# Jhuighuy/StormRuler

Measured on AMD Instinct MI355X. Metric: CG iterations/sec, 256^3 Poisson per GPU (+ SpMV achieved HBM GB/s in `roofline`), higher is better.
Workload: dtype f64

## Files before the change

### stormruler_amd/csrc/common.hpp

```cpp
#pragma once

#include <hip/hip_runtime.h>

#include <cstdint>
#include <cstdio>
#include <string>
#include <unordered_map>
#include <vector>

#include "../../include/storm_hip.h"

namespace storm {

void set_error(const char *fmt, ...) __attribute__((format(printf, 1, 2)));

#define STORM_FAIL(code, ...)        \
  do {                               \
    ::storm::set_error(__VA_ARGS__); \
    return (code);                   \
  } while (0)

#define STORM_REQUIRE(cond, ...) \
  do {                           \
    if (!(cond)) STORM_FAIL(STORM_HIP_E_INVALID, __VA_ARGS__); \
// ... 138 lines not shown
  int64_t opt_profile_spmv = 0;
  std::vector<storm::LazyStmt> lazy_q;
  std::unordered_map<const void *, int> occupancy;
  int64_t opt_test_disable = 0;
  int64_t opt_lazy = 0;
  int callback_depth = 0;
  int64_t n_lazy_fused_dots = 0, n_lazy_fused_pairs = 0, n_lazy_apply_dots = 0, n_lazy_cg_steps = 0;
  storm_hip_vec *lazy_spare = nullptr;
  int64_t opt_profile_comm = 0;
  int64_t opt_blas1_nt = 1;
  static constexpr int64_t opt_blas1_nt_rows = (int64_t)6 << 20;
  static constexpr int64_t opt_graph = 0;
  static constexpr int64_t opt_coop_mgs_min_rows = 0;
  int64_t opt_coop_mgs = 1;
  int64_t opt_latency_publish = 1;
  int64_t opt_coop_plain = 1;
  int64_t opt_coop_force_fail = 0;
  int coop_ran = 0;
  int coop_disabled = 0;
  int coop_fallback = 0;
  int64_t coop_skip = 0, coop_backoff = 0;
  int64_t opt_latency_path = 1;
  int64_t opt_resident_path = 1;
  static constexpr int64_t opt_resident_min_rows = 0;
  int64_t opt_resident_max_rows = (int64_t)1 << 22;
  int64_t opt_resident_planes = 0;
  static constexpr int64_t opt_resident_max_planes = 12;
  char *d_res_exch = nullptr;
  int64_t res_exch_rows = 0;
  int64_t opt_resident_profile = 0;
  long long *d_res_prof = nullptr;
  int res_prof_blocks = 0;
  char *d_res_slots = nullptr;
  int opt_lin_fuse = 1;
  int64_t opt_ticket_verify_inject = 0;
  int64_t opt_ticket_verify = 0;
  int opt_ticket_reduce = 1;
  int opt_fused_reduce = 1;
  int opt_latency_cache = 1;
  int64_t opt_latency_rows = 1 << 19;
  int64_t opt_rccl_fused = 1;
  int64_t opt_rccl_ticket = 1;
  int64_t opt_comm_wait_seconds = 120;
  int64_t opt_rccl_flag_wait = 1;
  int64_t opt_rccl_early_halo = 1;
  static constexpr int64_t opt_ipc_bicg_ticket = 1;
  static constexpr int64_t opt_ipc_fused = 1;
  static constexpr int64_t opt_ipc_streams = 2;
  int64_t opt_generic_solvers = 0;
  int64_t opt_cg_march_fill = 2048;
  int64_t opt_cg_march_alternate = 1;
  int64_t opt_cg_march = 8;
  int64_t opt_cg_residual_march = 1;
  int64_t opt_cg_fuse = 1;
  std::vector<std::pair<size_t, double *>> pool;
  struct VecArena {
    char *base = nullptr;
    size_t bytes = 0, pitch = 0;
    int slots = 0, used = 0;
  };
  std::vector<VecArena> arenas;
  int64_t opt_vec_arena = 1;
  static constexpr int64_t opt_vec_arena_contiguous = 1;
  static constexpr int64_t opt_cg_roles = 8;
  static constexpr int64_t opt_vec_arena_slots = 8;
  static constexpr int64_t opt_vec_arena_max_bytes = (int64_t)64 << 30;
  static constexpr int64_t opt_vec_arena_skew_kib = 0;
  size_t pool_bytes = 0;
  int64_t opt_pool_bytes = (int64_t)16 << 30;
  std::vector<hipEvent_t> prof_events;
  size_t prof_used = 0;
  const int *api_done = nullptr;
  int64_t n_resident_solves = 0, n_latency_solves = 0, n_throughput_solves = 0, n_engine_solves = 0, n_cg_fused_steps = 0;
  int64_t n_cg_residual_marches = 0;
  int64_t n_mgs_chain_steps = 0, n_mgs_quad_steps = 0;
  storm::Comm *comm = nullptr;
  int n_ranks = 1, rank = 0;
};

struct storm_hip_vec {
  storm_hip_ctx *ctx = nullptr;
  int64_t n_owned = 0, n_halo = 0;
  double *d = nullptr;
  double *base = nullptr;
  size_t bytes = 0;
  bool exposed = false;
};
constexpr int kVecGuard = 32;

namespace storm {

struct HaloPlan {
  int n_nbrs = 0;
  std::vector<int> nbr_rank;
  std::vector<int64_t> send_ptr, recv_ptr;
  int *d_send_idx = nullptr;
  double *d_sendbuf = nullptr;
  int64_t n_send = 0;
};

}

struct storm_hip_op {
  storm_hip_ctx *ctx = nullptr;
  int64_t n_rows = 0, n_halo = 0;
  int64_t n_slices = 0, n_interior_slices = 0;
  int64_t nnz = 0, ell_slots = 0, max_row_len = 0;
  int64_t *d_slice_off = nullptr;
  char *d_pack = nullptr;
  double *d_dict = nullptr;
  int dict_size = 0;
  int *d_offs = nullptr;
  int offs_size = 0;
  int xcd_group_sell = 0;
  int pair = 0;
  uint8_t *d_rec_idx = nullptr;
  uint64_t *d_rec_words = nullptr;
  int rec_words = 0;
  char *d_bnd_pack = nullptr;
  int bnd_width = 0;
  int canon_k = 0, canon_m1 = -1;
  int canon_off[7] = {0, 0, 0, 0, 0, 0, 0};
  int64_t pack_bytes = 0;
  int64_t spw = 1;
  int64_t tail_rows = 0, tail_nnz = 0;
  int *d_tail_row = nullptr;
  int64_t *d_tail_ptr = nullptr;
// ... 147 lines not shown
```

### stormruler_amd/csrc/context.hip

```cpp
#include <cstdarg>
#include <cstring>
#include <random>

#include <algorithm>
#include "common.hpp"

#include <cstddef>

namespace storm {

static thread_local char g_error[1024] = "";

void set_error(const char *fmt, ...) {
  va_list ap;
  va_start(ap, fmt);
  vsnprintf(g_error, sizeof g_error, fmt, ap);
  va_end(ap);
}

}

using namespace storm;

static void pool_release(storm_hip_ctx *c);
// ... 138 lines not shown
  else if (!strcmp(key, "coop_mgs_lds")) c->opt_coop_mgs_lds = value;
  else if (!strcmp(key, "coop_mgs_quad")) c->opt_coop_mgs_quad = value;
  else if (!strcmp(key, "cg_march_fill")) c->opt_cg_march_fill = value;
  else if (!strcmp(key, "resident_early")) c->opt_resident_early = value;
  else if (!strcmp(key, "mgs_steps")) c->opt_mgs_steps = value;
  else if (!strcmp(key, "vec_arena")) c->opt_vec_arena = value;
  else if (!strcmp(key, "spmv_mixed")) c->opt_spmv_mixed = value;
  else if (!strcmp(key, "spmv_canon_tile")) c->opt_spmv_canon_tile = value;
  else if (!strcmp(key, "spmv_canon_tile_min_rows")) c->opt_spmv_canon_tile_min_rows = value;
  else if (!strcmp(key, "fused_reduce")) c->opt_fused_reduce = (int)value;
  else if (!strcmp(key, "ticket_reduce")) c->opt_ticket_reduce = (int)value;
  else if (!strcmp(key, "ticket_verify")) c->opt_ticket_verify = value;
  else if (!strcmp(key, "ticket_verify_inject")) c->opt_ticket_verify_inject = value;
  else if (!strcmp(key, "lin_fuse")) c->opt_lin_fuse = (int)value;
  else if (!strcmp(key, "latency_rows")) c->opt_latency_rows = value;
  else if (!strcmp(key, "latency_cache")) c->opt_latency_cache = (int)value;
  else if (!strcmp(key, "nontemporal")) c->opt_nt = value;
  else if (!strcmp(key, "spmv_dict")) c->opt_spmv_dict = value;
  else if (!strcmp(key, "pool_bytes")) {
    c->opt_pool_bytes = value;
    if ((int64_t)c->pool_bytes > value || (value == 0 && !c->pool.empty())) {
      (void)hipStreamSynchronize(c->stream);
      pool_release(c);
    }
  }
  else if (!strcmp(key, "spmv_spw")) c->opt_spmv_spw = value;
  else if (!strcmp(key, "spmv_xcd_remap")) {
    STORM_REQUIRE(value >= 0 && value <= 4096, "ctx_set_option: spmv_xcd_remap %lld (0 .. 4096)", (long long)value);
    c->opt_spmv_xcd_remap = c->opt_spmv_xcd_remap_sell = value;
  }
  else if (!strcmp(key, "test_disable")) {
    c->opt_test_disable = value;
    c->opt_coop_mgs_apply = !(value & 1), c->opt_coop_mgs_prefetch = c->opt_coop_mgs_lds_prefetch = !(value & 2);
    c->opt_resident_apply_cache = !(value & 4), c->opt_resident_halo_interleave = !(value & 8);
    c->opt_latency_publish = !(value & 16), c->opt_coop_plain = !(value & 32), c->opt_cg_march_alternate = !(value & 64);
    c->opt_coop_mgs_xcd_runs = !(value & 128), c->opt_coop_mgs_alternate = !(value & 256);
    c->opt_coop_mgs_rotate_early = !(value & 512);
  }
  else if (!strcmp(key, "lazy_statements")) {
    if (value == 0) {
      STORM_TRY(lazy_sync(c));
      if (c->lazy_spare) (void)storm_hip_vec_destroy(c->lazy_spare), c->lazy_spare = nullptr;
    }
    c->opt_lazy = value;
  }
  else if (!strcmp(key, "profile_spmv")) c->opt_profile_spmv = value;
  else if (!strcmp(key, "profile_comm")) {
    c->opt_profile_comm = value;
    if (value != 0) STORM_TRY(comm_profile_reset(c));
  }
  else if (!strcmp(key, "cg_fuse")) c->opt_cg_fuse = value;
  else if (!strcmp(key, "cg_march")) c->opt_cg_march = value;
  else if (!strcmp(key, "cg_residual_march")) c->opt_cg_residual_march = value;
  else if (!strcmp(key, "spmv_record_index")) c->opt_spmv_record_index = value;
  else if (!strcmp(key, "blas1_nt")) c->opt_blas1_nt = value;
  else STORM_FAIL(STORM_HIP_E_INVALID, "ctx_set_option: unknown key '%s'", key);
  return STORM_HIP_OK;
}

int storm_hip_ctx_get_counter(storm_hip_ctx *c, const char *key, int64_t *value) {
  STORM_REQUIRE(c && key && value, "ctx_get_counter: null argument");
  if (!strcmp(key, "resident_solves")) *value = c->n_resident_solves;
  else if (!strcmp(key, "latency_solves")) *value = c->n_latency_solves;
  else if (!strcmp(key, "throughput_solves")) *value = c->n_throughput_solves;
  else if (!strcmp(key, "engine_solves")) *value = c->n_engine_solves;
  else if (!strcmp(key, "cg_fused_steps")) *value = c->n_cg_fused_steps;
  else if (!strcmp(key, "cg_residual_marches")) *value = c->n_cg_residual_marches;
  else if (!strcmp(key, "mgs_chain_steps")) *value = c->n_mgs_chain_steps;
  else if (!strcmp(key, "mgs_quad_steps")) *value = c->n_mgs_quad_steps;
  else if (!strcmp(key, "lazy_fused_dots")) *value = c->n_lazy_fused_dots;
  else if (!strcmp(key, "lazy_fused_pairs")) *value = c->n_lazy_fused_pairs;
  else if (!strcmp(key, "lazy_apply_dots")) *value = c->n_lazy_apply_dots;
  else if (!strcmp(key, "lazy_cg_steps")) *value = c->n_lazy_cg_steps;
  else if (!strcmp(key, "lazy_waiting")) *value = (int64_t)c->lazy_q.size();
  else if (!strncmp(key, "ipc_", 4)) {
    static const char *names[6] = {"ipc_allreduce_wait_ticks", "ipc_allreduces", "ipc_ack_wait_ticks", "ipc_ack_waits",
                                   "ipc_halo_slow_poll_ticks", "ipc_halo_slow_polls"};
    int k = -1;
    for (int i = 0; i < 6; ++i)
      if (!strcmp(key, names[i])) k = i;
    STORM_REQUIRE(k >= 0, "ctx_get_counter: unknown key '%s'", key);
    const long long v = comm_ipc_stat(c, k);
    STORM_REQUIRE(v >= 0, "ctx_get_counter: '%s' needs the peer-window transport", key);
    *value = v;
  }
  else if (!strncmp(key, "rccl_prof_", 10)) {
    static const char *names[8] = {"rccl_prof_exchanges", "rccl_prof_event_to_comm_ticks", "rccl_prof_pack_ticks",
                                   "rccl_prof_sendrecv_ticks", "rccl_prof_unhidden_wait_ticks", "rccl_prof_resume_ticks",
                                   "rccl_prof_allreduces", "rccl_prof_allreduce_ticks"};
    int k = -1;
    for (int i = 0; i < 8; ++i)
      if (!strcmp(key, names[i])) k = i;
    STORM_REQUIRE(k >= 0, "ctx_get_counter: unknown key '%s'", key);
    const long long v = comm_profile_read(c, k);
    STORM_REQUIRE(v >= 0, "ctx_get_counter: '%s' needs the RCCL transport with option profile_comm = 1", key);
    *value = v;
  }
  else if (!strncmp(key, "resident_phase_max_", 19) || !strncmp(key, "resident_phase_mean_", 20)) {
    const bool mx = key[15] == 'm' && key[16] == 'a';
    const int k = atoi(key + (mx ? 19 : 20));
    STORM_REQUIRE(c->d_res_prof != nullptr && c->res_prof_blocks > 0 && k >= 0 && k < 8, "ctx_get_counter: no resident profile (option resident_profile)");
    std::vector<long long> h((size_t)c->res_prof_blocks * 8);
    HIP_TRY(hipStreamSynchronize(c->stream));
    HIP_TRY(hipMemcpy(h.data(), c->d_res_prof, sizeof(long long) * h.size(), hipMemcpyDeviceToHost));
    long long m = 0, sum = 0;
    for (int b = 0; b < c->res_prof_blocks; ++b) m = std::max(m, h[(size_t)b * 8 + k]), sum += h[(size_t)b * 8 + k];
    *value = mx ? m : sum / c->res_prof_blocks;
  } else if (!strncmp(key, "resident_phase_block_", 21)) {
    int b = 0, k = 0;
    STORM_REQUIRE(sscanf(key + 21, "%d_%d", &b, &k) == 2 && c->d_res_prof != nullptr && b >= 0 && b < c->res_prof_blocks && k >= 0 && k < 8,
                  "ctx_get_counter: no such block / phase");
    long long v = 0;
    HIP_TRY(hipStreamSynchronize(c->stream));
    HIP_TRY(hipMemcpy(&v, c->d_res_prof + (size_t)b * 8 + k, sizeof v, hipMemcpyDeviceToHost));
    *value = v;
  }
  else STORM_FAIL(STORM_HIP_E_INVALID, "ctx_get_counter: unknown key '%s'", key);
  return STORM_HIP_OK;
}

// ... 395 lines not shown
```

### stormruler_amd/csrc/solver_device.hpp

```cpp
#pragma once

#include "common.hpp"
#include "ipc_device.hpp"
#include "wave_device.hpp"

namespace storm {

__device__ __forceinline__ double safe_divide(double x, double y) { return (y == 0.0) ? 0.0 : (x / y); }

__device__ inline void advance(SolverState *st, double abs_err) {
  st->absolute_error = abs_err;
  st->relative_error = abs_err / st->initial_error;
  bool conv = false;
  conv |= (st->abs_tol > 0.0) && (st->absolute_error < st->abs_tol);
  conv |= (st->rel_tol > 0.0) && (st->relative_error < st->rel_tol);
  st->iteration += 1;
  if (st->history) st->history[st->iteration] = abs_err;
  if (conv) st->converged = 1;
  if (conv || st->iteration >= st->num_iterations) st->done = 1;
  if (st->done_ring)
    __hip_atomic_store(st->done_ring + (st->iteration - 1) % kStateRing,
                       ring_word(st->ring_gen, (unsigned long long)st->iteration, st->done != 0), __ATOMIC_RELAXED,
                       __HIP_MEMORY_SCOPE_SYSTEM);
}

__device__ inline void begin(SolverState *st, double initial_error) {
  st->initial_error = initial_error;
  st->absolute_error = initial_error;
  st->relative_error = 0.0;
  st->iteration = 0;
  st->converged = 0;
  st->done = 0;
  if (st->history) st->history[0] = initial_error;
  if (st->abs_tol > 0.0 && initial_error < st->abs_tol) st->converged = 1, st->done = 1;
  if (st->num_iterations <= 0) st->done = 1;
  if (st->done && st->done_ring)
    for (int i = 0; i < kStateRing; ++i)
      __hip_atomic_store(st->done_ring + i, ring_word(st->ring_gen, kRingIterMask, true), __ATOMIC_RELAXED, __HIP_MEMORY_SCOPE_SYSTEM);
}

struct GmresDev {
  double *H, *beta, *cs, *sn;
  int m;
};
__device__ inline void gmres_givens_update(SolverState *st, GmresDev g, int k, double hn) {
  const int m = g.m;
#define H_(i, j) g.H[(i) * m + (j)]
  H_(k + 1, k) = hn;
  for (int i = 0; i < k; ++i) {
    const double chi = g.cs[i] * H_(i, k) + g.sn[i] * H_(i + 1, k);
    H_(i + 1, k) = -g.sn[i] * H_(i, k) + g.cs[i] * H_(i + 1, k);
    H_(i, k) = chi;
  }
  const double a = H_(k, k), b = H_(k + 1, k);
  const double rr = hypot(a, b);
  double cs, sn;
  if (rr > 0.0) cs = a / rr, sn = b / rr;
  else cs = 1.0, sn = 0.0;
  g.cs[k] = cs, g.sn[k] = sn;
  H_(k, k) = cs * H_(k, k) + sn * H_(k + 1, k);
  H_(k + 1, k) = 0.0;
  g.beta[k + 1] = -sn * g.beta[k];
  g.beta[k] *= cs;
  advance(st, fabs(g.beta[k + 1]));
#undef H_
}

__device__ __forceinline__ double block_sum256(double v, double *lds4) {
  v = wave_sum_down(v);
  const int lane = threadIdx.x & (kWave - 1), wave = threadIdx.x >> 6;
  __syncthreads();
  if (lane == 0) lds4[wave] = v;
  __syncthreads();
  return (lds4[0] + lds4[1]) + (lds4[2] + lds4[3]);
}

__device__ __forceinline__ double block_fold(const double *__restrict__ p, int i0, int i1, double *lds4) {
  double v = 0.0;
#pragma unroll 8
  for (int i = i0 + threadIdx.x; i < i1; i += kBlock) v += p[i];
  return block_sum256(v, lds4);
}
__device__ __forceinline__ double block_fold(const double *__restrict__ p, int n, double *lds4) {
  return block_fold(p, 0, n, lds4);
}

template <int K>
struct OutPtrs {
  double *p[K];
};

template <class Epi, int K>
__global__ __launch_bounds__(kBlock) void reduce_finish_kernel(const double *__restrict__ partials, int nblocks, int k,
                                                               OutPtrs<K> out, const int *done, IpcDev w, int use_ipc, Epi epi) {
  if (done && *done) return;
  __shared__ double lds4[4];
  __shared__ double vals[K];
  for (int j = 0; j < k; ++j) {
    const double sum = block_fold(partials + (int64_t)j * nblocks, nblocks, lds4);
    if (threadIdx.x == 0) vals[j] = sum;
  }
  if (use_ipc) ipc_allreduce_block(w, vals, k);
  else __syncthreads();
  if ((int)threadIdx.x < k) *out.p[threadIdx.x] = vals[threadIdx.x];
  __syncthreads();
  if (threadIdx.x == 0) epi();
}

template <class Epi, int K, class Tail>
int k_reduce_finish(storm_hip_ctx *c, const double *partials, int nblocks, int k, const OutPtrs<K> &out, const int *done,
                    const Epi &epi, const OutPtrs<K> &local, Tail rccl_tail) {
  STORM_TRY(k_reduce_stage1(c, &partials, &nblocks, k, done));
  IpcDev w{};
  const bool one = c->comm == nullptr || comm_ipc_next(c, &w);
  hipLaunchKernelGGL((reduce_finish_kernel<Epi, K>), dim3(1), dim3(kBlock), 0, c->stream, partials, nblocks, k, one ? out : local,
                     done, w, (int)(c->comm != nullptr && one), one ? epi : Epi{});
  HIP_TRY(hipGetLastError());
  return one ? STORM_HIP_OK : rccl_tail();
}

}
```

### stormruler_amd/csrc/solvers.hip

```cpp
#include <algorithm>
#include <cmath>
#include <cstddef>
#include <cstring>

#include "common.hpp"
#include "blas1_device.hpp"
#include "wave_device.hpp"
#include "solver_device.hpp"
#include "ticket_device.hpp"
#include "ipc_device.hpp"
#include "spmv_device.hpp"

namespace storm {

enum Slot {
  S_GAMMA = 0, S_PZ, S_GAMMA_NEW, S_BETA, S_ALPHA,
  S_RHO, S_RTV, S_TR, S_TT, S_OMEGA, S_RR, S_RHO_NEW,
  S_TMP, S_HN,
  S_SCRATCH = 32,
  S_ALPHA_SEEN = 48,
};

enum StepKind {
  STEP_NONE = 0,
// ... 265 lines not shown
      el[u] = 0.0;
      if (lane == 0) el[u] = one_at(row - 1);
      if (lane == kWave - 1) el[u] = one_at(row + 2);
    }
#pragma unroll
    for (int u = 0; u < kUnroll; ++u) {
      const int64_t i = base + u * kBlock;
      double2v xg[6];
      xg[0] = nb[u][0], xg[1] = nb[u][1], xg[4] = nb[u][2], xg[5] = nb[u][3];
      const double left = dpp_shift<0x138>(c[u].y);
      const double right = dpp_shift<0x130>(c[u].x);
      xg[2].x = lane == 0 ? el[u] : left;
      xg[2].y = c[u].x;
      xg[3].x = c[u].y;
      xg[3].y = lane == kWave - 1 ? el[u] : right;
      const double2v vz = lattice_pair_apply(dict_sh, rec_word<IDX>(w[u], words_sh), xg, c[u], op_alpha, op_beta);
      if (i < n2) {
        vr[u] -= alpha * vz;
        r2[i] = vr[u];
        acc += vr[u].x * vr[u].x;
        acc += vr[u].y * vr[u].y;
      }
    }
  }
  cg_r_finish(st, acc, bx, nullptr, tickets, IpcDev{}, 0, lds4);
}

static bool cg_r_recompute_applies(const storm_hip_op *op, bool tick) {
  storm_hip_ctx *c = op->ctx;
  MarchArgs M;
  int nb = 0;
  return c->opt_cg_residual_march != 0 && tick && c->comm == nullptr && c->opt_ticket_verify == 0 && op->n_rows % 2 == 0 &&
         spmv_can_march(op) && cg_march_geometry(op, &M, &nb);
}
static int cg_r_recompute_run(const storm_hip_op *op, int nbv, Scal alpha, Scal beta, const double *p, SolverState *st, double *r,
                              const double *pz_partials, int n_pz, int reverse) {
  storm_hip_ctx *c = op->ctx;
  CanonTileArgs T;
  int nbt = 0;
  STORM_REQUIRE(canon_tile_geometry(op, &T, &nbt), "cg: the residual recompute needs a lattice operator");
  const SellArgs A = lattice_args(op);
  const size_t lds = sizeof(uint64_t) * (size_t)A.rec_words_n;
  const TicketArgs tk{c->d_tickets, c->d_partials, c->d_ticket_sums};
  if (A.rec_idx != nullptr)
    hipLaunchKernelGGL(cg_r_recompute_kernel<true>, dim3(nbv), dim3(kBlock), lds, c->stream, op->n_rows, st, r, p, A, T, alpha,
                       beta, pz_partials, n_pz, reverse, tk);
  else
    hipLaunchKernelGGL(cg_r_recompute_kernel<false>, dim3(nbv), dim3(kBlock), lds, c->stream, op->n_rows, st, r, p, A, T, alpha,
                       beta, pz_partials, n_pz, reverse, tk);
  HIP_TRY(hipGetLastError());
  return STORM_HIP_OK;
}

constexpr int kUnrollXp = 1;
__global__ __launch_bounds__(kBlock) void cg_xp_kernel(int64_t n, const SolverState *st, long long my_iteration,
                                                       double *__restrict__ x, double *__restrict__ p,
                                                       const double *__restrict__ r, int nt, int reverse) {
  if (st->iteration < my_iteration) return;
  const unsigned bx = reverse ? gridDim.x - 1 - blockIdx.x : blockIdx.x;
  const bool update_p = !st->done && r != nullptr;
  const double alpha = st->s[S_ALPHA], beta = st->s[S_BETA];
  const int64_t n2 = n >> 1;
  double2v *x2 = reinterpret_cast<double2v *>(x), *p2 = reinterpret_cast<double2v *>(p);
  const double2v *r2 = reinterpret_cast<const double2v *>(r);
  nt_dispatch(nt, [&](auto nt) {
  for (int64_t base = (int64_t)bx * (kBlock * kUnrollXp) + threadIdx.x; base < n2;
       base += (int64_t)gridDim.x * (kBlock * kUnrollXp)) {
    double2v vx[kUnrollXp], vp[kUnrollXp], vr[kUnrollXp];
#pragma unroll
    for (int u = 0; u < kUnrollXp; ++u) {
      const int64_t i = base + u * kBlock;
      if (i < n2) {
        vx[u] = ldv(x2 + i, nt), vp[u] = ldv(p2 + i, nt);
        if (update_p) vr[u] = ldv(r2 + i, nt);
      }
    }
#pragma unroll
    for (int u = 0; u < kUnrollXp; ++u) {
      const int64_t i = base + u * kBlock;
      if (i < n2) {
        vx[u] += alpha * vp[u];
        stv(x2 + i, vx[u], nt);
        if (update_p) stv(p2 + i, vr[u] + beta * vp[u], nt);
      }
    }
  }
  });
  if ((n & 1) && bx == 0 && threadIdx.x == 0) {
    const int64_t i = n - 1;
    x[i] += alpha * p[i];
    if (update_p) p[i] = r[i] + beta * p[i];
  }
}
static inline int xp_blocks(int64_t n) {
  int64_t b = ((n >> 1) + kBlock * kUnrollXp - 1) / (kBlock * kUnrollXp);
  return (int)(b < 1 ? 1 : (b > 131072 ? 131072 : b));
}

template <bool SECOND>
__global__ __launch_bounds__(kBlock) void bicg_update_kernel(int64_t n, SolverState *st, double *__restrict__ x,
                                                             double *__restrict__ r, const double *__restrict__ p,
                                                             const double *__restrict__ w,
                                                             const double *__restrict__ rt,
                                                             double *__restrict__ partials, int nt, int reverse,
                                                             TicketArgs tickets, const double *r_in = nullptr,
                                                             IpcDev ipc_w = IpcDev{}, int use_ipc = 0) {
// ... 739 lines not shown
  double *history = args.history;
  storm_hip_ctx *c = op->ctx;
  HIP_TRY(hipSetDevice(c->device));
  const int64_t n = op->n_rows;
  Driver d{c, op, alpha, beta, n, c->d_state, &c->d_state->done};
  STORM_TRY(prepare_state(d, params, history));
  VecPool pool;
  if (res_eligible(op, false)) {
    bool taken = false;
    STORM_TRY(res_solve(false, op, alpha, beta, b->d, x->d, nullptr, c->d_state, &taken));
    if (taken) return ++c->n_resident_solves, collect(d, result, history, applies_cg, 0);
  }
  if (cg_latency_eligible(op)) {
    STORM_TRY(pool.make(x, 2));
    bool taken = false;
    STORM_TRY(cg_latency_solve(op, alpha, beta, b->d, x->d, pool.v[0]->d, pool.v[1]->d, c->d_state, &taken));
    if (taken) return ++c->n_latency_solves, collect(d, result, history, applies_cg, 0);
  }
  ++c->n_throughput_solves;
  const size_t v0 = pool.v.size();
  const bool may_fuse_step = c->opt_cg_fuse != 0 && spmv_can_fuse_cg(op);
  STORM_TRY(pool.make(x, may_fuse_step ? 4 : 3, false));
  int role[4] = {0, 1, 2, 3};
  for (int64_t k = 0; k < c->opt_cg_roles % 24; ++k) std::next_permutation(role, role + 4);
  if (!may_fuse_step) role[0] = 0, role[1] = 1, role[2] = 2;
  double *p = pool.v[v0 + role[0]]->d, *r = pool.v[v0 + role[1]]->d, *z = pool.v[v0 + role[2]]->d;
  const int nbv = vec_blocks(c, n);

  int nb = 0;
  STORM_TRY(d.apply(x->d, r, nullptr, false, &nb, false));
  hipLaunchKernelGGL(init_residual_kernel, dim3(nbv), dim3(kBlock), 0, c->stream, n, r, b->d, p, c->d_partials,
                     stream_nt(c, n));
  HIP_TRY(hipGetLastError());
  {
    const int slots[1] = {S_GAMMA};
    STORM_TRY(d.finish(nbv, 1, slots, STEP_CG_INIT, true));
  }
  int64_t cur_it = 0;
  const bool sweep = c->opt_sweep_alternate != 0;
  const int nt_stream = (int)(stream_nt(c, n) != 0 && !(sweep && c->opt_sweep_alternate == 2));
  IpcDev ipc_w{};
  const bool ipc = c->comm != nullptr && comm_ipc_next(c, &ipc_w);
  const bool tick = c->opt_ticket_reduce != 0 && (c->comm == nullptr || ipc) && nbv <= kTicketGroup * kTicketMaxGroups;
  const bool tick_spmv = tick && !ipc && 4 * (int64_t)spmv_grid_blocks(op) <= kSinglePassPartials;
  const bool rccl = c->comm != nullptr && comm_is_rccl(c);
  const bool fuse_step = c->opt_cg_fuse != 0 && spmv_can_fuse_cg(op) &&
                         (rccl ? true : ((c->comm == nullptr || ipc) && tick && !tick_spmv));
  const bool rtick = rccl && fuse_step && c->opt_ticket_reduce != 0 && c->opt_rccl_ticket != 0 &&
                     nbv <= kTicketGroup * kTicketMaxGroups;
  double *p_alt = nullptr;
  if (fuse_step) p_alt = pool.v[v0 + role[3]]->d, ++c->n_cg_fused_steps;
  const bool r_march = fuse_step && !rccl && cg_r_recompute_applies(op, tick);
  if (r_march) ++c->n_cg_residual_marches;
  int64_t last_enqueued = -1;
  auto enqueue_iteration = [&]() -> int {
    const int q = fuse_step ? 0 : sweep ? (int)(cur_it & 1) : 0;
    c->spmv_reverse = q;
    int pz_done = 0;
    int st_apply;
    const bool r_march_now = r_march && cur_it > 0;
    if (fuse_step && cur_it > 0) {
      const Driver::CgStep step{(long long)cur_it, x->d, r, p_alt};
      st_apply = d.apply(p, r_march_now ? nullptr : z, p, false, &nb, true, -1, -1, &pz_done, &step);
      std::swap(p, p_alt);
    } else {
      st_apply = d.apply(p, z, p, false, &nb, true, tick_spmv ? (int)S_PZ : -1, -1, &pz_done);
    }
    last_enqueued = cur_it;
    c->spmv_reverse = 0;
    STORM_TRY(st_apply);
    const double *pz_partials = nullptr;
    if (pz_done) {
    } else if (nb == 0) {
      const double *bs[1] = {z};
      STORM_TRY(k_multi_dot(c, p, bs, 1, n, d.slot(S_PZ), d.done));
      if (c->comm != nullptr) STORM_TRY(comm_allreduce_sum(c, d.slot(S_PZ), 1));
    } else if (rtick && (int64_t)nb + kStage2 <= c->partials_capacity) {
      hipLaunchKernelGGL(reduce_stage1_ticket_kernel<1>, dim3(kStage2), dim3(kBlock), 0, c->stream, c->d_partials, nb,
                         d.slot(S_PZ), d.st, TicketArgs{c->d_tickets, c->d_partials + nb, c->d_ticket_sums}, ipc_w, 0);
      HIP_TRY(hipGetLastError());
      STORM_TRY(comm_allreduce_sum(c, d.slot(S_PZ), 1));
    } else if (tick && (nb > kSinglePassPartials || ipc) && (int64_t)nb + kStage2 <= c->partials_capacity) {
      hipLaunchKernelGGL(reduce_stage1_ticket_kernel<1>, dim3(kStage2), dim3(kBlock), 0, c->stream, c->d_partials, nb,
                         d.slot(S_PZ), d.st, TicketArgs{c->d_tickets, c->d_partials + nb, c->d_ticket_sums}, ipc_w, (int)ipc);
      HIP_TRY(hipGetLastError());
    } else if (c->comm == nullptr && nb > kSinglePassPartials) {
      pz_partials = c->d_partials;
      STORM_TRY(k_reduce_stage1(c, &pz_partials, &nb, 1, d.done));
    } else {
      const int slots[1] = {S_PZ};
      STORM_TRY(d.finish(nb, 1, slots, STEP_NONE));
    }
    if (r_march_now) {
      STORM_TRY(cg_r_recompute_run(op, nbv, host_scal(alpha), host_scal(beta), p, d.st, r, pz_partials, (int)kStage2, sweep ? 1 - q : 0));
    } else {
      hipLaunchKernelGGL(cg_r_kernel, dim3(nbv), dim3(kBlock), 0, c->stream, n, d.st, r, z, c->d_partials,
                         nt_stream, pz_partials, (int)kStage2, sweep ? 1 - q : 0,
                         (tick || rtick) ? TicketArgs{c->d_tickets, c->d_partials, c->d_ticket_sums} : TicketArgs{nullptr, nullptr, nullptr},
                         ipc_w, rtick ? 2 : (int)(ipc && tick));
      HIP_TRY(hipGetLastError());
    }
    if (rtick) {
      STORM_TRY(comm_allreduce_sum(c, d.slot(S_GAMMA_NEW), 1));
      hipLaunchKernelGGL(step_kernel, dim3(1), dim3(1), 0, c->stream, (int)STEP_CG_RR, d.st, d.g, false);
      HIP_TRY(hipGetLastError());
    } else if (!tick) {
      const int slots[1] = {S_GAMMA_NEW};
      STORM_TRY(d.finish(nbv, 1, slots, STEP_CG_RR));
    }
    if (tick && c->opt_ticket_verify > 0 && cur_it % c->opt_ticket_verify == 0) {
      STORM_TRY(d.verify(p, z, nullptr, S_PZ, -1, (long long)(cur_it + 1)));
      STORM_TRY(d.verify(r, r, nullptr, S_GAMMA, -1, (long long)(cur_it + 1)));
    }
    if (fuse_step) return STORM_HIP_OK;
    if (rccl && c->opt_rccl_early_halo != 0 && op->halo.n_nbrs > 0)
      STORM_TRY(comm_halo_exchange_begin_formed(op, 2, r, p, nullptr, d.slot(S_BETA), nullptr, p));
    hipLaunchKernelGGL(cg_xp_kernel, dim3(xp_blocks(n)), dim3(kBlock), 0, c->stream, n, d.st, (long long)(cur_it + 1), x->d,
                       p, r, nt_stream, q);
    HIP_TRY(hipGetLastError());
    return STORM_HIP_OK;
  };
  for (int64_t it = 0; it < params->num_iterations; ++it) {
    cur_it = it;
    STORM_TRY(enqueue_iteration());
    bool stop = false;
    STORM_TRY(post_and_poll(d, it, &stop));
    if (stop) break;
  }
  if (fuse_step && last_enqueued >= 0) {
    hipLaunchKernelGGL(cg_xp_kernel, dim3(xp_blocks(n)), dim3(kBlock), 0, c->stream, n, d.st, (long long)(last_enqueued + 1),
                       x->d, p, (const double *)nullptr, nt_stream, 0);
    HIP_TRY(hipGetLastError());
  }
  comm_forget_prebegun(c);
  return collect(d, result, history, applies_cg, 0);
}

int solve_bicgstab_body(const FusedSolveArgs &args) {
  const storm_hip_op *op = args.op;
  const double alpha = args.alpha, beta = args.beta;
  const storm_hip_vec *b = args.b;
  storm_hip_vec *x = args.x;
  const storm_hip_solver_params *params = args.params;
  storm_hip_solver_result *result = args.result;
  double *history = args.history;
  storm_hip_ctx *c = op->ctx;
// ... 278 lines not shown
```

### stormruler_amd/csrc/ticket_device.hpp

```cpp
#pragma once
#include "common.hpp"
#include "wave_device.hpp"

namespace storm {

constexpr int kTicketGroup = 64;
constexpr int kTicketStride = 16;
constexpr int kTicketMaxGroups = 2048;
static_assert(kMaxStreamBlocks <= kTicketGroup * kTicketMaxGroups, "stream_blocks() may exceed the ticket counters");

struct TicketArgs {
  int *cnt;
  double *part1;
  double *part2;
};

template <int KMAX>
__device__ __forceinline__ void ticket_publish(double *p, size_t stride, const double (&v)[KMAX], int k) {
  unsigned long long seen = 0ull;
#pragma unroll
  for (int j = 0; j < KMAX; ++j) {
    if (j < k) {
#ifdef STORM_TICKET_STORE_EXPERIMENT
      __hip_atomic_store(p + (size_t)j * stride, v[j], __ATOMIC_RELAXED, __HIP_MEMORY_SCOPE_AGENT);
#else
      seen ^= __hip_atomic_exchange(reinterpret_cast<unsigned long long *>(p + (size_t)j * stride),
                                    (unsigned long long)__double_as_longlong(v[j]), __ATOMIC_RELAXED,
                                    __HIP_MEMORY_SCOPE_AGENT);
#endif
    }
  }
#ifdef STORM_TICKET_STORE_EXPERIMENT
  __builtin_amdgcn_fence(__ATOMIC_RELEASE, "workgroup");
#endif
  asm volatile("" : : "v"(seen) : "memory");
}
__device__ __forceinline__ double ticket_wave_sum(double v) {
  return wave_sum_all(v);
}

template <int KMAX>
__device__ __forceinline__ bool ticket_reduce_wave0(const TicketArgs &t, const double (&mine)[KMAX], int k, unsigned bx,
                                                    unsigned nb, double (&total)[KMAX]) {
  const unsigned lane = threadIdx.x & (kWave - 1);
  const unsigned g = bx / kTicketGroup, ng = (nb + kTicketGroup - 1) / kTicketGroup;
  const unsigned gsize = (nb - g * kTicketGroup) < (unsigned)kTicketGroup ? (nb - g * kTicketGroup) : (unsigned)kTicketGroup;
  int go = 0;
  if (lane == 0) {
    ticket_publish<KMAX>(t.part1 + bx, nb, mine, k);
    int *c = t.cnt + (size_t)(1 + g) * kTicketStride;
    if (__hip_atomic_fetch_add(c, 1, __ATOMIC_RELAXED, __HIP_MEMORY_SCOPE_AGENT) == (int)gsize - 1) {
      __hip_atomic_store(c, 0, __ATOMIC_RELAXED, __HIP_MEMORY_SCOPE_AGENT);
      go = 1;
    }
  }
  go = __shfl(go, 0, kWave);
  if (!go) return false;
  double gp[KMAX];
#pragma unroll
  for (int j = 0; j < KMAX; ++j) {
    gp[j] = 0.0;
    if (j < k && lane < gsize)
      gp[j] = __hip_atomic_load(t.part1 + (size_t)j * nb + (size_t)g * kTicketGroup + lane, __ATOMIC_RELAXED, __HIP_MEMORY_SCOPE_AGENT);
  }
#pragma unroll
  for (int j = 0; j < KMAX; ++j) gp[j] = ticket_wave_sum(gp[j]);
  go = 0;
  if (lane == 0) {
    ticket_publish<KMAX>(t.part2 + g, ng, gp, k);
    if (__hip_atomic_fetch_add(t.cnt, 1, __ATOMIC_RELAXED, __HIP_MEMORY_SCOPE_AGENT) == (int)ng - 1) {
      __hip_atomic_store(t.cnt, 0, __ATOMIC_RELAXED, __HIP_MEMORY_SCOPE_AGENT);
      go = 1;
    }
  }
  go = __shfl(go, 0, kWave);
  if (!go) return false;
  constexpr int kAhead = KMAX <= 4 ? 4 : 2;
#pragma unroll
  for (int j = 0; j < KMAX; ++j) total[j] = 0.0;
  for (unsigned i0 = lane; i0 < ng; i0 += kWave * kAhead) {
    double v[KMAX][kAhead];
#pragma unroll
    for (int j = 0; j < KMAX; ++j)
#pragma unroll
      for (int u = 0; u < kAhead; ++u) {
        const unsigned i = i0 + u * kWave;
        v[j][u] = 0.0;
        if (j < k && i < ng) v[j][u] = __hip_atomic_load(t.part2 + (size_t)j * ng + i, __ATOMIC_RELAXED, __HIP_MEMORY_SCOPE_AGENT);
      }
#pragma unroll
    for (int j = 0; j < KMAX; ++j)
#pragma unroll
      for (int u = 0; u < kAhead; ++u)
        if (i0 + u * kWave < ng) total[j] += v[j][u];
  }
#pragma unroll
  for (int j = 0; j < KMAX; ++j) total[j] = ticket_wave_sum(total[j]);
  return true;
}

}
```

Measured before the change: 5065.

## Add z-plane chunked residual-march kernel with multi-slot ticket reduction

Adds a CG residual-update kernel in which each block marches through a chunk of consecutive z-planes. It keeps the previous, current and next planes of p in registers and LDS, so the stencil reuses p across planes instead of re-gathering it. Per-plane partial sums of r·r are folded into the existing two-level ticket reduction through a new slot-aware variant that lets one wave publish many block slots. This cuts the number of blocks and the per-block reduction overhead, at the cost of fewer blocks in flight and more LDS and register pressure. The path is on by default whenever the canonical tile geometry applies.

```diff
diff --git a/stormruler_amd/csrc/common.hpp b/stormruler_amd/csrc/common.hpp
--- a/stormruler_amd/csrc/common.hpp
+++ b/stormruler_amd/csrc/common.hpp
@@ -214,6 +214,9 @@
   int64_t opt_cg_march_alternate = 1;
   int64_t opt_cg_march = 8;
   int64_t opt_cg_residual_march = 1;
+  int64_t opt_cg_residual_planes = 1;
+  int64_t opt_cg_residual_chunk = 16;
+  int64_t opt_cg_residual_fill = 512;
   int64_t opt_cg_fuse = 1;
   std::vector<std::pair<size_t, double *>> pool;
   struct VecArena {
@@ -235,6 +238,7 @@
   const int *api_done = nullptr;
   int64_t n_resident_solves = 0, n_latency_solves = 0, n_throughput_solves = 0, n_engine_solves = 0, n_cg_fused_steps = 0;
   int64_t n_cg_residual_marches = 0;
+  int64_t n_cg_residual_plane_marches = 0;
   int64_t n_mgs_chain_steps = 0, n_mgs_quad_steps = 0;
   storm::Comm *comm = nullptr;
   int n_ranks = 1, rank = 0;
diff --git a/stormruler_amd/csrc/context.hip b/stormruler_amd/csrc/context.hip
--- a/stormruler_amd/csrc/context.hip
+++ b/stormruler_amd/csrc/context.hip
@@ -214,6 +214,9 @@
   else if (!strcmp(key, "cg_fuse")) c->opt_cg_fuse = value;
   else if (!strcmp(key, "cg_march")) c->opt_cg_march = value;
   else if (!strcmp(key, "cg_residual_march")) c->opt_cg_residual_march = value;
+  else if (!strcmp(key, "cg_residual_planes")) c->opt_cg_residual_planes = value;
+  else if (!strcmp(key, "cg_residual_chunk")) c->opt_cg_residual_chunk = value;
+  else if (!strcmp(key, "cg_residual_fill")) c->opt_cg_residual_fill = value;
   else if (!strcmp(key, "spmv_record_index")) c->opt_spmv_record_index = value;
   else if (!strcmp(key, "blas1_nt")) c->opt_blas1_nt = value;
   else STORM_FAIL(STORM_HIP_E_INVALID, "ctx_set_option: unknown key '%s'", key);
@@ -228,6 +231,7 @@
   else if (!strcmp(key, "engine_solves")) *value = c->n_engine_solves;
   else if (!strcmp(key, "cg_fused_steps")) *value = c->n_cg_fused_steps;
   else if (!strcmp(key, "cg_residual_marches")) *value = c->n_cg_residual_marches;
+  else if (!strcmp(key, "cg_residual_plane_marches")) *value = c->n_cg_residual_plane_marches;
   else if (!strcmp(key, "mgs_chain_steps")) *value = c->n_mgs_chain_steps;
   else if (!strcmp(key, "mgs_quad_steps")) *value = c->n_mgs_quad_steps;
   else if (!strcmp(key, "lazy_fused_dots")) *value = c->n_lazy_fused_dots;
diff --git a/stormruler_amd/csrc/solver_device.hpp b/stormruler_amd/csrc/solver_device.hpp
--- a/stormruler_amd/csrc/solver_device.hpp
+++ b/stormruler_amd/csrc/solver_device.hpp
@@ -66,13 +66,14 @@
 #undef H_
 }
 
+__device__ __forceinline__ double block_sum256_of_waves(const double *lds4) { return (lds4[0] + lds4[1]) + (lds4[2] + lds4[3]); }
 __device__ __forceinline__ double block_sum256(double v, double *lds4) {
   v = wave_sum_down(v);
   const int lane = threadIdx.x & (kWave - 1), wave = threadIdx.x >> 6;
   __syncthreads();
   if (lane == 0) lds4[wave] = v;
   __syncthreads();
-  return (lds4[0] + lds4[1]) + (lds4[2] + lds4[3]);
+  return block_sum256_of_waves(lds4);
 }
 
 __device__ __forceinline__ double block_fold(const double *__restrict__ p, int i0, int i1, double *lds4) {
diff --git a/stormruler_amd/csrc/solvers.hip b/stormruler_amd/csrc/solvers.hip
--- a/stormruler_amd/csrc/solvers.hip
+++ b/stormruler_amd/csrc/solvers.hip
@@ -341,6 +341,179 @@
   return STORM_HIP_OK;
 }
 
+struct ResidualPlanesArgs {
+  int a, b;
+  int runs_per_plane;
+  int per_xcd;
+  int planes;
+  int nz;
+  int max_gather;
+};
+constexpr int kResidualMaxChunk = 32;
+template <int HLP, bool IDX>
+__global__ __launch_bounds__(kBlock) void cg_r_planes_kernel(SolverState *st, double *__restrict__ r, const double *__restrict__ p,
+                                                             SellArgs A, ResidualPlanesArgs G, Scal alpha_s, Scal beta_s,
+                                                             const double *__restrict__ pz_partials, int n_pz, int reverse,
+                                                             TicketArgs tickets) {
+  const int done = st->done;
+  __shared__ double lds4[4];
+  __shared__ double dict_sh[32];
+  __shared__ double wave_part[kResidualMaxChunk * (kBlock / kWave)];
+  extern __shared__ __attribute__((aligned(16))) double plane_sh[];
+  const int a = G.a, b = G.b;
+  const int ldw = kStreamBlockElems + 2 * a;
+  unsigned long long *words_sh = reinterpret_cast<unsigned long long *>(plane_sh + 2 * ldw);
+  const int lane = threadIdx.x & (kWave - 1);
+  const int wave = __builtin_amdgcn_readfirstlane(threadIdx.x >> 6);
+  const int bidx = reverse ? (int)(gridDim.x - 1 - blockIdx.x) : (int)blockIdx.x;
+  int zc, yt;
+  if (G.per_xcd > 0) {
+    const int xcd = bidx & (kNumXcd - 1), j = bidx >> 3;
+    zc = j / G.per_xcd;
+    yt = xcd * G.per_xcd + (j - zc * G.per_xcd);
+  } else {
+    zc = bidx / G.runs_per_plane;
+    yt = bidx - zc * G.runs_per_plane;
+  }
+  const int z_begin = zc * G.nz, z_end = min(z_begin + G.nz, G.planes), nz = z_end - z_begin;
+  auto plane = [&](int s) { return z_begin + s; };
+  const int p0 = yt * kStreamBlockElems;
+  const char *pg = reinterpret_cast<const char *>(p) - (size_t)kVecGuard * 8;
+  double2v *r2 = reinterpret_cast<double2v *>(r);
+
+  struct Flight {
+    double2v p[kUnroll], hp[HLP];
+  };
+  int hat[HLP], hjj[HLP];
+#pragma unroll
+  for (int i = 0; i < HLP; ++i) {
+    const int h = (int)threadIdx.x + kBlock * i;
+    hjj[i] = 2 * h < a ? 2 * h - a : kStreamBlockElems + 2 * h - a;
+    hat[i] = h < a ? a + hjj[i] : -1;
+  }
+  auto load_p = [&](int64_t row) {
+    int64_t gi = row + kVecGuard;
+    gi = gi < 0 ? 0 : (gi > (int64_t)G.max_gather ? (int64_t)G.max_gather : gi);
+    return *reinterpret_cast<const double2v *>(pg + (size_t)gi * 8);
+  };
+  auto issue_p = [&](int zp, bool own, Flight &f) {
+    const int64_t row0 = (int64_t)zp * b + p0;
+#pragma unroll
+    for (int u = 0; u < kUnroll; ++u) f.p[u] = load_p(row0 + 2 * ((int)threadIdx.x + kBlock * u));
+#pragma unroll
+    for (int i = 0; i < HLP; ++i) {
+      f.hp[i] = double2v{0.0, 0.0};
+      if (own && hat[i] >= 0) f.hp[i] = load_p(row0 + hjj[i]);
+    }
+  };
+  auto issue_rw = [&](int zp, double2v (&vr)[kUnroll], RecRaw<IDX> (&w)[kUnroll]) {
+    const int64_t row0 = (int64_t)zp * b + p0;
+#pragma unroll
+    for (int u = 0; u < kUnroll; ++u) {
+      const int64_t row = row0 + 2 * ((int)threadIdx.x + kBlock * u);
+      vr[u] = r2[row >> 1];
+      w[u] = rec_load<IDX>(A, (uint32_t)row);
+    }
+  };
+
+  Flight cur, nxt, fl;
+  double2v pm[kUnroll], vr[kUnroll];
+  RecRaw<IDX> w[kUnroll];
+  issue_p(plane(-1), false, fl);
+#pragma unroll
+  for (int u = 0; u < kUnroll; ++u) pm[u] = fl.p[u];
+  issue_p(plane(0), true, cur);
+  issue_rw(plane(0), vr, w);
+  issue_p(plane(1), 1 < nz, nxt);
+  if (threadIdx.x < 32) dict_sh[threadIdx.x] = A.dict[threadIdx.x];
+  if (IDX) rec_table_fill(A, words_sh);
+  if (done) return;
+  const double alpha = cg_r_alpha(st, pz_partials, n_pz, lds4);
+  const double op_alpha = ld_scal2(alpha_s), op_beta = ld_scal2(beta_s);
+  for (int s = 0; s < nz; ++s) {
+    const int zp = plane(s);
+    double *buf = plane_sh + (s & 1) * ldw;
+#pragma unroll
+    for (int u = 0; u < kUnroll; ++u) *reinterpret_cast<double2v *>(&buf[a + 2 * ((int)threadIdx.x + kBlock * u)]) = cur.p[u];
+#pragma unroll
+    for (int i = 0; i < HLP; ++i)
+      if (hat[i] >= 0) *reinterpret_cast<double2v *>(&buf[hat[i]]) = cur.hp[i];
+    double2v vrn[kUnroll];
+    RecRaw<IDX> wn[kUnroll];
+    if (s + 2 <= nz) issue_p(plane(s + 2), s + 2 < nz, fl);
+    if (s + 1 < nz) issue_rw(plane(s + 1), vrn, wn);
+    __syncthreads();
+    const int64_t i0 = (((int64_t)zp * b + p0) >> 1) + threadIdx.x;
+    double acc = 0.0;
+#pragma unroll
+    for (int u = 0; u < kUnroll; ++u) {
+      const int at = a + 2 * ((int)threadIdx.x + kBlock * u);
+      double2v xg[6];
+      march_neighbours(buf, at, a, lane, pm[u], nxt.p[u], cur.p[u], xg);
+      const double2v vz = lattice_pair_apply(dict_sh, rec_word<IDX>(w[u], words_sh), xg, cur.p[u], op_alpha, op_beta);
+      vr[u] -= alpha * vz;
+      r2[i0 + u * kBlock] = vr[u];
+      acc += vr[u].x * vr[u].x;
+      acc += vr[u].y * vr[u].y;
+    }
+    acc = wave_sum_down(acc);
+    if (lane == 0) wave_part[s * (kBlock / kWave) + wave] = acc;
+#pragma unroll
+    for (int u = 0; u < kUnroll; ++u) pm[u] = cur.p[u], vr[u] = vrn[u], w[u] = wn[u];
+    cur = nxt, nxt = fl;
+  }
+  __syncthreads();
+  if (threadIdx.x >= kWave) return;
+  const bool on = lane < nz;
+  const double mine = on ? block_sum256_of_waves(wave_part + lane * (kBlock / kWave)) : 0.0;
+  const unsigned bxv = on ? (unsigned)(plane(lane) * G.runs_per_plane + yt) : 0u;
+  double total;
+  if (ticket_reduce_wave0_slots(tickets, mine, on, bxv, (unsigned)(G.planes * G.runs_per_plane), &total) && threadIdx.x == 0) {
+    st->s[S_GAMMA_NEW] = total;
+    do_step(STEP_CG_RR, st, GmresDev{});
+  }
+}
+
+static bool cg_r_planes_geometry(const storm_hip_op *op, ResidualPlanesArgs *G, int *n_blocks) {
+  storm_hip_ctx *c = op->ctx;
+  CanonTileArgs T;
+  int nbt = 0;
+  if (c->opt_cg_residual_planes == 0 || !canon_tile_geometry(op, &T, &nbt)) return false;
+  const int64_t n = op->n_rows;
+  if (T.b % kStreamBlockElems != 0 || n % T.b != 0 || n / kStreamBlockElems > kMaxStreamBlocks) return false;
+  if ((int64_t)sizeof(double) * 2 * (kStreamBlockElems + 2 * T.a) + (int64_t)sizeof(uint64_t) * op->rec_words > 60 * 1024) return false;
+  G->a = T.a, G->b = T.b, G->max_gather = T.max_gather;
+  G->runs_per_plane = T.b / kStreamBlockElems;
+  G->per_xcd = (G->runs_per_plane % kNumXcd == 0 && c->opt_spmv_xcd_remap != 0) ? G->runs_per_plane / kNumXcd : 0;
+  G->planes = (int)(n / T.b);
+  const int64_t zc = std::min<int64_t>(std::max<int64_t>(c->opt_cg_residual_chunk, 2), kResidualMaxChunk);
+  const int64_t want = c->opt_cg_residual_fill;
+  const int64_t fill = want > 0 ? (int64_t)G->planes * G->runs_per_plane / want : zc;
+  G->nz = (int)std::min<int64_t>(std::min<int64_t>(zc, std::max<int64_t>(2, fill)), G->planes);
+  *n_blocks = ((G->planes + G->nz - 1) / G->nz) * G->runs_per_plane;
+  return true;
+}
+static int cg_r_planes_run(const storm_hip_op *op, const ResidualPlanesArgs &G, int n_blocks, Scal alpha, Scal beta, const double *p,
+                           SolverState *st, double *r, const double *pz_partials, int n_pz, int reverse) {
+  storm_hip_ctx *c = op->ctx;
+  const SellArgs A = lattice_args(op);
+  const size_t lds = sizeof(double) * 2 * (size_t)(kStreamBlockElems + 2 * G.a) + sizeof(uint64_t) * (size_t)A.rec_words_n;
+  const TicketArgs tk{c->d_tickets, c->d_partials, c->d_ticket_sums};
+#define PLANES_GO(HLP_, IX_)                                                                                                   \
+  hipLaunchKernelGGL((cg_r_planes_kernel<HLP_, IX_>), dim3(n_blocks), dim3(kBlock), lds, c->stream, st, r, p, A, G, alpha, beta, \
+                     pz_partials, n_pz, reverse, tk)
+  if (G.a <= kBlock) {
+    if (A.rec_idx != nullptr) PLANES_GO(1, true);
+    else PLANES_GO(1, false);
+  } else {
+    if (A.rec_idx != nullptr) PLANES_GO(2, true);
+    else PLANES_GO(2, false);
+  }
+#undef PLANES_GO
+  HIP_TRY(hipGetLastError());
+  return STORM_HIP_OK;
+}
+
 constexpr int kUnrollXp = 1;
 __global__ __launch_bounds__(kBlock) void cg_xp_kernel(int64_t n, const SolverState *st, long long my_iteration,
                                                        double *__restrict__ x, double *__restrict__ p,
@@ -1186,6 +1359,10 @@
   if (fuse_step) p_alt = pool.v[v0 + role[3]]->d, ++c->n_cg_fused_steps;
   const bool r_march = fuse_step && !rccl && cg_r_recompute_applies(op, tick);
   if (r_march) ++c->n_cg_residual_marches;
+  ResidualPlanesArgs r_planes_args;
+  int r_planes_blocks = 0;
+  const bool r_planes = r_march && cg_r_planes_geometry(op, &r_planes_args, &r_planes_blocks);
+  if (r_planes) ++c->n_cg_residual_plane_marches;
   int64_t last_enqueued = -1;
   auto enqueue_iteration = [&]() -> int {
     const int q = fuse_step ? 0 : sweep ? (int)(cur_it & 1) : 0;
@@ -1225,7 +1402,10 @@
       const int slots[1] = {S_PZ};
       STORM_TRY(d.finish(nb, 1, slots, STEP_NONE));
     }
-    if (r_march_now) {
+    if (r_march_now && r_planes) {
+      STORM_TRY(cg_r_planes_run(op, r_planes_args, r_planes_blocks, host_scal(alpha), host_scal(beta), p, d.st, r, pz_partials,
+                                (int)kStage2, sweep ? 1 - q : 0));
+    } else if (r_march_now) {
       STORM_TRY(cg_r_recompute_run(op, nbv, host_scal(alpha), host_scal(beta), p, d.st, r, pz_partials, (int)kStage2, sweep ? 1 - q : 0));
     } else {
       hipLaunchKernelGGL(cg_r_kernel, dim3(nbv), dim3(kBlock), 0, c->stream, n, d.st, r, z, c->d_partials,
diff --git a/stormruler_amd/csrc/ticket_device.hpp b/stormruler_amd/csrc/ticket_device.hpp
--- a/stormruler_amd/csrc/ticket_device.hpp
+++ b/stormruler_amd/csrc/ticket_device.hpp
@@ -40,6 +40,32 @@
 }
 
 template <int KMAX>
+__device__ __forceinline__ void ticket_fold_groups(const TicketArgs &t, int k, unsigned ng, double (&total)[KMAX]) {
+  const unsigned lane = threadIdx.x & (kWave - 1);
+  constexpr int kAhead = KMAX <= 4 ? 4 : 2;
+#pragma unroll
+  for (int j = 0; j < KMAX; ++j) total[j] = 0.0;
+  for (unsigned i0 = lane; i0 < ng; i0 += kWave * kAhead) {
+    double v[KMAX][kAhead];
+#pragma unroll
+    for (int j = 0; j < KMAX; ++j)
+#pragma unroll
+      for (int u = 0; u < kAhead; ++u) {
+        const unsigned i = i0 + u * kWave;
+        v[j][u] = 0.0;
+        if (j < k && i < ng) v[j][u] = __hip_atomic_load(t.part2 + (size_t)j * ng + i, __ATOMIC_RELAXED, __HIP_MEMORY_SCOPE_AGENT);
+      }
+#pragma unroll
+    for (int j = 0; j < KMAX; ++j)
+#pragma unroll
+      for (int u = 0; u < kAhead; ++u)
+        if (i0 + u * kWave < ng) total[j] += v[j][u];
+  }
+#pragma unroll
+  for (int j = 0; j < KMAX; ++j) total[j] = ticket_wave_sum(total[j]);
+}
+
+template <int KMAX>
 __device__ __forceinline__ bool ticket_reduce_wave0(const TicketArgs &t, const double (&mine)[KMAX], int k, unsigned bx,
                                                     unsigned nb, double (&total)[KMAX]) {
   const unsigned lane = threadIdx.x & (kWave - 1);
@@ -75,27 +101,78 @@
   }
   go = __shfl(go, 0, kWave);
   if (!go) return false;
-  constexpr int kAhead = KMAX <= 4 ? 4 : 2;
+  ticket_fold_groups<KMAX>(t, k, ng, total);
+  return true;
+}
+
+__device__ __forceinline__ bool ticket_reduce_wave0_slots(const TicketArgs &t, double mine, bool on, unsigned bxv, unsigned nb,
+                                                          double *total) {
+  const unsigned lane = threadIdx.x & (kWave - 1);
+  const unsigned g = bxv / kTicketGroup, ng = (nb + kTicketGroup - 1) / kTicketGroup;
+  const unsigned gsize = (nb - g * kTicketGroup) < (unsigned)kTicketGroup ? (nb - g * kTicketGroup) : (unsigned)kTicketGroup;
+  if (on) {
+    const double v[1] = {mine};
+    ticket_publish<1>(t.part1 + bxv, nb, v, 1);
+  }
+  int count = 0;
+  bool leader = false;
+  for (unsigned long long rest = __ballot(on); rest != 0ull;) {
+    const int first = __ffsll((long long)rest) - 1;
+    const unsigned long long same = __ballot(on && g == (unsigned)__shfl((int)g, first, kWave));
+    if ((int)lane == first) leader = true, count = __popcll(same);
+    rest &= ~same;
+  }
+  int go = 0;
+  if (leader) {
+    int *c = t.cnt + (size_t)(1 + g) * kTicketStride;
+    if (__hip_atomic_fetch_add(c, count, __ATOMIC_RELAXED, __HIP_MEMORY_SCOPE_AGENT) + count == (int)gsize) {
+      __hip_atomic_store(c, 0, __ATOMIC_RELAXED, __HIP_MEMORY_SCOPE_AGENT);
+      go = 1;
+    }
+  }
+  unsigned long long fin = __ballot(go != 0);
+  if (fin == 0ull) return false;
+  const int n_fin = __popcll(fin);
+  double gsum = 0.0;
+  while (fin != 0ull) {
+    int at[4];
+    double gp[4];
 #pragma unroll
-  for (int j = 0; j < KMAX; ++j) total[j] = 0.0;
-  for (unsigned i0 = lane; i0 < ng; i0 += kWave * kAhead) {
-    double v[KMAX][kAhead];
+    for (int j = 0; j < 4; ++j) {
+      at[j] = fin != 0ull ? __ffsll((long long)fin) - 1 : -1;
+      if (at[j] >= 0) fin &= fin - 1ull;
+    }
 #pragma unroll
-    for (int j = 0; j < KMAX; ++j)
+    for (int j = 0; j < 4; ++j) {
+      gp[j] = 0.0;
+      if (at[j] >= 0) {
+        const unsigned gj = (unsigned)__shfl((int)g, at[j], kWave), nj = (unsigned)__shfl((int)gsize, at[j], kWave);
+        if (lane < nj)
+          gp[j] = __hip_atomic_load(t.part1 + (size_t)gj * kTicketGroup + lane, __ATOMIC_RELAXED, __HIP_MEMORY_SCOPE_AGENT);
+      }
+    }
 #pragma unroll
-      for (int u = 0; u < kAhead; ++u) {
-        const unsigned i = i0 + u * kWave;
-        v[j][u] = 0.0;
-        if (j < k && i < ng) v[j][u] = __hip_atomic_load(t.part2 + (size_t)j * ng + i, __ATOMIC_RELAXED, __HIP_MEMORY_SCOPE_AGENT);
-      }
-#pragma unroll
-    for (int j = 0; j < KMAX; ++j)
-#pragma unroll
-      for (int u = 0; u < kAhead; ++u)
-        if (i0 + u * kWave < ng) total[j] += v[j][u];
+    for (int j = 0; j < 4; ++j) {
+      const double sj = ticket_wave_sum(gp[j]);
+      if ((int)lane == at[j]) gsum = sj;
+    }
   }
-#pragma unroll
-  for (int j = 0; j < KMAX; ++j) total[j] = ticket_wave_sum(total[j]);
+  if (go) {
+    const double v[1] = {gsum};
+    ticket_publish<1>(t.part2 + g, ng, v, 1);
+  }
+  go = 0;
+  if (lane == 0) {
+    if (__hip_atomic_fetch_add(t.cnt, n_fin, __ATOMIC_RELAXED, __HIP_MEMORY_SCOPE_AGENT) + n_fin == (int)ng) {
+      __hip_atomic_store(t.cnt, 0, __ATOMIC_RELAXED, __HIP_MEMORY_SCOPE_AGENT);
+      go = 1;
+    }
+  }
+  go = __shfl(go, 0, kWave);
+  if (!go) return false;
+  double tot[1];
+  ticket_fold_groups<1>(t, 1, ng, tot);
+  *total = tot[0];
   return true;
 }
 
```

Measured after the change: 5410, median of 6. 1.07x the previous value.
